# yoxu515/aot-benchmark

Measured on NVIDIA H100. Metric: frames/sec (480p, 10 obj), higher is better.
Workload: dtype f32

## Files before the change

### aot_benchmark_b200/csrc/local_attn.cu

```cuda
#include "common.cuh"

namespace aotb {

constexpr int LW = 15, LR = 7, LTAPS = 225;

__device__ __forceinline__ void cp_async16(float* dst_smem, const float* src, int bytes) {
    asm volatile("cp.async.ca.shared.global [%0], [%1], 16, %2;" ::"r"((uint32_t)__cvta_generic_to_shared(dst_smem)), "l"(src),
                 "r"(bytes) : "memory");
}
__device__ __forceinline__ void cp_async_wait_all() { asm volatile("cp.async.commit_group;\n\tcp.async.wait_group 0;" ::: "memory"); }

struct LocalArgs {
    const float* q; int ldq;
    const float* k; int ldk;
    const float* v; int ldv;
    const float* relk_w;
    const float* relk_b;
    const float* relv;
    float* out; int ldo;
    int h, w, H;
    float T;
};

template <int D, int DV, bool HAS_RELV, bool STAGE_WK>
__global__ void __launch_bounds__(256) local_attn_kernel(const LocalArgs p) {
    pdl_sync();
    constexpr int WARPS = 8;
    constexpr int WKS = D + 4;
    extern __shared__ __align__(16) float smem[];
    float* q_raw = smem;
    float* q_scl = q_raw + WARPS * D;
    float* prob = q_scl + WARPS * D;
    float* wk_s = prob + WARPS * 232;
    float* relv_s = wk_s + (STAGE_WK ? LTAPS * WKS : 0);

    const int g = blockIdx.y;
    const int warp = threadIdx.x >> 5, lane = threadIdx.x & 31;
    const int N = p.h * p.w;
    const int qi = blockIdx.x * WARPS + warp;

    if constexpr (STAGE_WK) {
        const float* src = p.relk_w + (size_t)g * LTAPS * D;
        for (int f = threadIdx.x; f < LTAPS * (D / 4); f += blockDim.x) {
            const int r = f / (D / 4), c = (f % (D / 4)) * 4;
            *reinterpret_cast<float4*>(wk_s + r * WKS + c) = __ldg(reinterpret_cast<const float4*>(src + r * D + c));
        }
    }
    if constexpr (HAS_RELV) {
        const float* src = p.relv + (size_t)g * DV * LTAPS;
        for (int f = threadIdx.x; f < DV * LTAPS; f += blockDim.x) relv_s[f] = __ldg(src + f);
    }
    if (qi < N) {
        for (int c = lane; c < D; c += 32) {
// ... 250 lines not shown
    }
    cp_async_wait_all();
    __syncthreads();

    {
        const int ly = warp / (TX / 3), lx0 = (warp % (TX / 3)) * 3;
        float acc[3] = {0.f, 0.f, 0.f};
#pragma unroll 1
        for (int dy = 0; dy < LW; ++dy) {
            const float* vrow = halo + ((ly + dy) * HWD + lx0) * LD + lane;
            float vv[LW + 2], rr[LW];
#pragma unroll
            for (int j = 0; j < LW + 2; ++j) vv[j] = vrow[j * LD];
#pragma unroll
            for (int dx = 0; dx < LW; ++dx) rr[dx] = rvs[(dy * LW + dx) * D + lane];
#pragma unroll
            for (int i = 0; i < 3; ++i) {
                const float4* pp = reinterpret_cast<const float4*>(prob + (ly * TX + lx0 + i) * PLD + dy * 16);
                const float4 p0 = pp[0], p1 = pp[1], p2 = pp[2], p3 = pp[3];
                const float pa[16] = {p0.x, p0.y, p0.z, p0.w, p1.x, p1.y, p1.z, p1.w,
                                      p2.x, p2.y, p2.z, p2.w, p3.x, p3.y, p3.z, p3.w};
#pragma unroll
                for (int dx = 0; dx < LW; ++dx) acc[i] = fmaf(pa[dx], vv[i + dx] + rr[dx], acc[i]);
            }
        }
        const int y = ty0 + ly;
#pragma unroll
        for (int i = 0; i < 3; ++i) {
            const int x = tx0 + lx0 + i;
            if (y < p.h && x < p.w) p.out[(size_t)(y * p.w + x) * p.ldo + g * D + lane] = acc[i];
        }
    }
}

static int launch_local_tile(const LocalArgs& a, const float* relv_t, cudaStream_t st) {
    constexpr int TY = 8, TX = 6;
    const size_t smem = sizeof(float) * (size_t)((TY + 14) * (TX + 14) * 36 + TY * TX * 32 + TY * TX * LW * 16 + LTAPS * 32);
    static bool configured = false;
    if (!configured) {
        cudaError_t e = cudaFuncSetAttribute(local_attn_tile_kernel<TY, TX>, cudaFuncAttributeMaxDynamicSharedMemorySize,
                                             (int)smem);
        if (e != cudaSuccess) {
            set_error("aotb_local_attention_tile_f32: cudaFuncSetAttribute: %s", cudaGetErrorString(e));
            return AOTB_ERR_CUDA;
        }
        configured = true;
    }
    dim3 grid(cdiv(a.h, TY) * cdiv(a.w, TX), a.H);
    launch(local_attn_tile_kernel<TY, TX>, dim3(grid), dim3(512), smem, st, a, relv_t);
    return check_launch("aotb_local_attention_tile_f32");
}


template <int TY, int TX, int KC, int VC>
__global__ void __launch_bounds__(512, 1) local_gated_tile_kernel(const LocalArgs p) {
    pdl_sync();
    constexpr int C = 32, HH = TY + 2 * LR, HWD = TX + 2 * LR, NPOS = HH * HWD, LD = 36;
    constexpr int NT = 512, NQ = TY * TX, PLD = LW * 16, DQ = KC * C;
    static_assert(TX % 3 == 0 && TY * (TX / 3) == NT / 32, "aggregate pass: one warp per 3 queries");
    static_assert(LW * HWD <= NT && 2 * LTAPS <= NT && NQ % 2 == 0, "pass mappings");
    extern __shared__ __align__(16) float smem[];
    float* halo = smem;
    float* qs = halo + NPOS * LD;
    float* prob = qs + NQ * DQ;

    const int tid = threadIdx.x, warp = tid >> 5, lane = tid & 31;
    const int tiles_x = (p.w + TX - 1) / TX;
    const int ty0 = (blockIdx.x / tiles_x) * TY, tx0 = (blockIdx.x % tiles_x) * TX;
    const int cg = blockIdx.y;

    auto load_halo = [&](const float* src, int ld, int c0) {
        for (int f = tid; f < NPOS * 8; f += NT) {
            const int pos = f >> 3, c4 = (f & 7) * 4;
            const int hy = pos / HWD, hx = pos - hy * HWD;
            const int yy = ty0 - LR + hy, xx = tx0 - LR + hx;
            const bool in = yy >= 0 && yy < p.h && xx >= 0 && xx < p.w;
            cp_async16(halo + pos * LD + c4, in ? src + (size_t)(yy * p.w + xx) * ld + c0 + c4 : src, in ? 16 : 0);
        }
    };
    for (int f = tid; f < NQ * (DQ / 4); f += NT) {
        const int ql = f / (DQ / 4), c4 = (f % (DQ / 4)) * 4;
        const int ly = ql / TX, lx = ql - ly * TX;
        const int y = ty0 + ly, x = tx0 + lx;
        float4 v = make_float4(0.f, 0.f, 0.f, 0.f);
        if (y < p.h && x < p.w) v = __ldg(reinterpret_cast<const float4*>(p.q + (size_t)(y * p.w + x) * p.ldq + c4));
        *reinterpret_cast<float4*>(qs + ql * DQ + c4) = v;
    }
    load_halo(p.k, p.ldk, 0);
    cp_async_wait_all();
    __syncthreads();

    if (tid < 2 * LTAPS) {
        const int half = tid / LTAPS, tap = tid - half * LTAPS;
        const float bias = __ldg(p.relk_b + tap);
        const int slot = (tap / LW) * 16 + tap % LW;
#pragma unroll 1
        for (int kc = 0; kc < KC; ++kc) {
            float wk[C];
            const float4* wp = reinterpret_cast<const float4*>(p.relk_w + (size_t)tap * DQ + kc * C);
#pragma unroll
            for (int c = 0; c < C / 4; ++c) {
                const float4 t = __ldg(wp + c);
                wk[4 * c] = t.x; wk[4 * c + 1] = t.y; wk[4 * c + 2] = t.z; wk[4 * c + 3] = t.w;
            }
#pragma unroll 2
            for (int qi = 0; qi < NQ / 2; ++qi) {
// ... 124 lines not shown

static int launch_local_gated_tile(const LocalArgs& a, cudaStream_t st) {
    constexpr int TY = 8, TX = 6, KC = 4, VC = 8;
    const size_t smem = sizeof(float) * (size_t)((TY + 14) * (TX + 14) * 36 + TY * TX * KC * 32 + TY * TX * LW * 16);
    static bool configured = false;
    if (!configured) {
        cudaError_t e = cudaFuncSetAttribute(local_gated_tile_kernel<TY, TX, KC, VC>, cudaFuncAttributeMaxDynamicSharedMemorySize,
                                             (int)smem);
        if (e != cudaSuccess) {
            set_error("aotb_local_gated_tile_f32: cudaFuncSetAttribute: %s", cudaGetErrorString(e));
            return AOTB_ERR_CUDA;
        }
        configured = true;
    }
    dim3 grid(cdiv(a.h, TY) * cdiv(a.w, TX), 1024 / (VC * 32));
    launch(local_gated_tile_kernel<TY, TX, KC, VC>, dim3(grid), dim3(512), smem, st, a);
    return check_launch("aotb_local_gated_tile_f32");
}

}

using namespace aotb;

extern "C" int aotb_local_attention_f32(const float* q, int ldq, const float* k, int ldk, const float* v, int ldv,
                                        const float* relk_w, const float* relk_b, const float* relv, float* out,
                                        int ldo, int h, int w, int H, int d_att, int d_v, void* stream) {
    AOTB_REQUIRE(q && k && v && relk_w && relk_b && out && h > 0 && w > 0 && H > 0,
                 "aotb_local_attention_f32: bad args");
    AOTB_REQUIRE(ldq % 4 == 0 && ldk % 4 == 0 && ldv % 4 == 0 && ldo % 4 == 0, "aotb_local_attention_f32: ld %% 4");
    LocalArgs a;
    a.q = q; a.ldq = ldq; a.k = k; a.ldk = ldk; a.v = v; a.ldv = ldv;
    a.relk_w = relk_w; a.relk_b = relk_b; a.relv = relv; a.out = out; a.ldo = ldo;
    a.h = h; a.w = w; a.H = H; a.T = sqrtf((float)d_att);
    cudaStream_t st = (cudaStream_t)stream;
    if (d_att == 32 && d_v == 32 && relv) return launch_local<32, 32, true, true>(a, st);
    if (d_att == 128 && d_v == 1024 && !relv) return launch_local<128, 1024, false, false>(a, st);
    set_error("aotb_local_attention_f32: unsupported head shape d_att=%d d_v=%d relv=%d", d_att, d_v, relv != nullptr);
    return AOTB_ERR_UNSUPPORTED;
}

extern "C" int aotb_local_attention_tile_f32(const float* q, int ldq, const float* k, int ldk, const float* v, int ldv,
                                             const float* relk_w, const float* relk_b, const float* relv_t, float* out,
                                             int ldo, int h, int w, int H, void* stream) {
    AOTB_REQUIRE(q && k && v && relk_w && relk_b && relv_t && out && h > 0 && w > 0 && H > 0,
                 "aotb_local_attention_tile_f32: bad args");
    AOTB_REQUIRE(ldq % 4 == 0 && ldk % 4 == 0 && ldv % 4 == 0, "aotb_local_attention_tile_f32: ld %% 4");
    LocalArgs a;
    a.q = q; a.ldq = ldq; a.k = k; a.ldk = ldk; a.v = v; a.ldv = ldv;
    a.relk_w = relk_w; a.relk_b = relk_b; a.relv = nullptr; a.out = out; a.ldo = ldo;
    a.h = h; a.w = w; a.H = H; a.T = sqrtf(32.f);
    return launch_local_tile(a, relv_t, (cudaStream_t)stream);
}

extern "C" int aotb_local_gated_tile_f32(const float* q, int ldq, const float* k, int ldk, const float* v, int ldv,
                                         const float* relk_w, const float* relk_b, float* out, int ldo, int h, int w,
                                         void* stream) {
    AOTB_REQUIRE(q && k && v && relk_w && relk_b && out && h > 0 && w > 0, "aotb_local_gated_tile_f32: bad args");
    AOTB_REQUIRE(ldq % 4 == 0 && ldk % 4 == 0 && ldv % 4 == 0, "aotb_local_gated_tile_f32: ld %% 4");
    LocalArgs a;
    a.q = q; a.ldq = ldq; a.k = k; a.ldk = ldk; a.v = v; a.ldv = ldv;
    a.relk_w = relk_w; a.relk_b = relk_b; a.relv = nullptr; a.out = out; a.ldo = ldo;
    a.h = h; a.w = w; a.H = 1; a.T = sqrtf(128.f);
    return launch_local_gated_tile(a, (cudaStream_t)stream);
}
```

### aot_benchmark_b200/engine.py

```python
from __future__ import annotations

import functools
import math

import numpy as np
import torch
import torch.nn as nn

from . import ops
from .plan import get_plan

A_NONE, A_RELU, A_GELU, A_SILU, A_RELU6 = ops.ACT_NONE, ops.ACT_RELU, ops.ACT_GELU, ops.ACT_SILU, ops.ACT_RELU6
A_HSWISH = ops.ACT_HSWISH

LT_PROBE = None
import os as _os
LT_IMPL = _os.environ.get("AOTB_LT_IMPL", "tc_exact")
LOCAL_IMPL = _os.environ.get("AOTB_LOCAL_IMPL", "tile")
DEAOT_LT = _os.environ.get("AOTB_DEAOT_LT", "tc")
SHARD_XCHG = _os.environ.get("AOTB_SHARD_XCHG", "nccl")
SHARD_SMAX = 16
SUB_ENGINE_STREAMS = _os.environ.get("AOTB_SUB_ENGINE_STREAMS", "1") == "1"
SHARD_GRAPHS = _os.environ.get("AOTB_SHARD_GRAPHS", "1") == "1"


def _symm_alloc(numel, device, group):
    import torch.distributed as dist
    import torch.distributed._symmetric_memory as symm_mem
    t = symm_mem.empty(numel, dtype=torch.float32, device=device)
    hdl = symm_mem.rendezvous(t, group if group is not None else dist.group.WORLD)
    return hdl, (lambda r, sizes, off: hdl.get_buffer(r, sizes, torch.float32, off))


GEMM_GROW_FRAMES = int(_os.environ.get("AOTB_GEMM_GROW_FRAMES", "8"))
_LT_NAMES = {"simt": "attn_f32_kernel<32,32> (fp32 SIMT flash attention)",
             "tc_exact": "attn_tc_kernel<1,1> (wgmma fp16x2 exact: 6+8 MMAs per 64-key tile)",
             "tc_fast": "attn_tc_kernel<1,1> (wgmma fp16 fast: 2+4 MMAs per 64-key tile)"}
_DEAOT_LT_NAMES = {"simt": "attn_f32_kernel<128,256> (fp32 SIMT flash attention, DeAOT 1 x 128 / 1024 head)",
                   "gemm": "conv_tc_kernel (Q K^T) -> row_softmax_kernel -> conv_tc_kernel (P V): wgmma GEMMs over split-fp16 "
                           "copies of the bank (deaot_lt.cu)",
                   "tc": "attn_tc_kernel<4,2> (fused wgmma flash attention, 128 queries x 64 value channels per CTA)"}


def deaot_lt_kernel_name():
    return _DEAOT_LT_NAMES.get(DEAOT_LT, DEAOT_LT)


LT_KERNEL_NAME = _LT_NAMES.get(LT_IMPL, LT_IMPL) + (f", layout '{ops.LT_VARIANT}'" if LT_IMPL.startswith("tc") else "")


USE_GRAPHS = _os.environ.get("AOTB_GRAPHS", "1") == "1"
USE_PDL = _os.environ.get("AOTB_PDL", "1") == "1"
CONV_TILING = _os.environ.get("AOTB_CONV_TILING", "model")
_CONV_TILING_MASK = {"model": 0, "narrow": 1}


def _apply_pdl():
    from ._lib import lib, check
    lib().aotb_set_pdl(1 if USE_PDL else 0)
    check(lib().aotb_set_conv_tiling(_CONV_TILING_MASK[CONV_TILING]), "aotb_set_conv_tiling")
BANK_INIT_FRAMES = int(_os.environ.get("AOTB_BANK_FRAMES", "24"))
OFFLINE_ENC_CHUNK = 16


def _resolve_mem_max(aot_model, long_term_mem_max):
    m = getattr(aot_model.cfg, "TEST_LONG_TERM_MEM_MAX", None) if long_term_mem_max is None else long_term_mem_max
    if m is None:
        return None
    if int(m) != m or m < 2:
        raise ValueError(f"long_term_mem_max must be an integer >= 2 (the first memory frame and at least one recent one), got {m}")
    return int(m)
# ... 951 lines not shown
        for li in range(self._plan().L):
            ops.bank_append(K_src[li], self.bank_K[li], 0, offset_dev=off, stream=st)
            ops.bank_append(V_src[li], self.bank_V[li], 0, offset_dev=off, stream=st)
            if self._tc:
                ops.tc_pack_rows(K_src[li], self.bank_Kp[li], 0, row_off_dev=off, stream=st)
                ops.tc_pack_rows(V_src[li], self.bank_Vp[li], 0, row_off_dev=off, stream=st)
            if self._gemm_lt:
                ops.split_rows(K_src[li], self.bank_Kh[li], self.bank_Kl[li], row_off_dev=off, stream=st)
                ops.split_cols(V_src[li], self.bank_VhT[li], self.bank_VlT[li], col_off_dev=off, stream=st)
            if getattr(self, "_gp_tc", False):
                ops.tc_pack_rows(K_src[li], self.bank_gpK[li], 0, row_off_dev=off, stream=st)
                ops.tc_pack_rows(V_src[li], self.bank_gpV[li], 0, row_off_dev=off, stream=st)
        ops.counter_add(off, N, stream=st)

    def _latest_kv(self):
        return self._new_K, self._new_V

    def _lstt_forward(self, embs, id_emb, st):
        P = self._plan()
        ws = self._ws
        N, C, H = self.enc_hw, P.C, P.H
        h, w = self.enc_size_2d
        d = C // H
        proj = embs.nhwc[-1].view(N, C)
        ops.eltwise(ops.EW_COPY, proj, None, ws.x, stream=st)
        ops.eltwise(ops.EW_COPY, proj, None, ws.cat[:, :C], stream=st)
        x = ws.x
        is_ref = id_emb is not None
        if is_ref:
            stK, stV = self._next_short_slot()
        else:
            stK, stV = self.st_K, self.st_V
        for li in range(P.L):
            Lw = P.layers[li]
            ops.layernorm(x, Lw.norm1[0], Lw.norm1[1], ws.ln, add=self.pos_emb, out2=ws.ln_pos, stream=st)
            ops.linear(ws.ln_pos, Lw.sa_qk_w, Lw.sa_qk_b, ws.qk, stream=st)
            ops.linear(ws.ln, Lw.sa_v_w, Lw.sa_v_b, ws.v, stream=st)
            if self._tc:
                self._tc_attention(ws.qk[:, :C], ws.qk[:, C:], ws.v, None, None, N, ws.core[:, :C], st)
            else:
                ops.attention(ws.qk[:, :C], ws.qk[:, C:], ws.v, ws.core[:, :C], H, d, d, Tk=N, stream=st)
            ops.linear(ws.core[:, :C], Lw.sa_proj_w, Lw.sa_proj_b, x, res=x, stream=st)
            cQ, cV = self.curr_Q[li], self.curr_V[li]
            ops.layernorm(x, Lw.norm2[0], Lw.norm2[1], cV, stream=st)
            ops.linear(cV, Lw.linQ_w, Lw.linQ_b, cQ, stream=st)
            if is_ref:
                ops.eltwise(ops.EW_ADD, cV, id_emb, ws.tmp, stream=st)
                ops.linear(ws.tmp, Lw.linV_w, Lw.linV_b, stV[li], stream=st)
                ops.eltwise(ops.EW_COPY, cQ, None, stK[li], stream=st)
                gK, gV, Tk = stK[li], stV[li], N
            else:
                gK, gV, Tk = self.bank_K[li], self.bank_V[li], self.bank_len
            self._long_term_attention(li, cQ, gK, gV, Tk, ws.core[:, :C], st)
            if d == 32 and LOCAL_IMPL == "tile":
                ops.local_attention_tile(cQ, stK[li], stV[li], Lw.relk_w, Lw.relk_b, Lw.relv_t, ws.core[:, C:], h, w, H,
                                         stream=st)
            else:
                ops.local_attention(cQ, stK[li], stV[li], Lw.relk_w, Lw.relk_b, Lw.relv, ws.core[:, C:], h, w, H, d, d,
                                    stream=st)
            ops.linear(ws.core, Lw.lst_proj_w, Lw.lst_proj_b, x, res=x, stream=st)
            ops.layernorm(x, Lw.norm3[0], Lw.norm3[1], ws.ln, stream=st)
            ops.linear(ws.ln, Lw.lin1_w, Lw.lin1_b, ws.ff, stream=st)
            ops.groupnorm(ws.ff.view(1, N, 4 * C), Lw.gn[0], Lw.gn[1], ws.ff.view(1, N, 4 * C), 32, A_GELU, ws.gn_ws,
                          stream=st)
            ops.dwconv(ws.ff.view(1, h, w, 4 * C), Lw.dw_w, None, ws.ff2.view(1, h, w, 4 * C), K=5, pad=2, stream=st)
            ops.linear(ws.ff2, Lw.lin2_w, Lw.lin2_b, x, res=x, stream=st)
            ops.layernorm(x, Lw.dec_norm[0], Lw.dec_norm[1], ws.cat[:, (li + 1) * C:(li + 2) * C], stream=st)
        if is_ref:
            self._commit_short_slot(stK, stV)
        self._have_lstt = True

    def _long_term_attention(self, li, Q, K, V, Tk, out, st):
        P = self._plan()
        d = P.C // P.H
        probe = LT_PROBE
        use_tc = self._tc and (K is self.bank_K[li])
        if use_tc:
            ops.tc_pack_rows(Q, self._ws.Qp, 0, div=math.sqrt(d), stream=st)
        if probe is not None:
            e0, e1 = torch.cuda.Event(enable_timing=True), torch.cuda.Event(enable_timing=True)
            e0.record()
        if use_tc and self.kv_shard is not None:
            self._sharded_attention(li, out, st)
        elif self.kv_shard is not None and K is self.bank_K[li]:
            raise ops.AotbError("sharded long-term bank needs the tensor-core attention kernel (8 heads x 32); this model's "
                                "head shape runs on the fp32 kernel, which has no partial (m, l, O) outputs")
        elif use_tc and self._usage():
            self._usage_attention(li, self._ws.Qp, self.bank_Kp[li], self.bank_Vp[li], out, st)
        elif use_tc:
            self._tc_attention(None, None, None, self.bank_Kp[li], self.bank_Vp[li], Tk, out, st, Tk_dev=self.tk_dev)
        elif self._tc:
            self._tc_attention(Q, K, V, None, None, Tk, out, st)
        else:
            ops.attention(Q, K, V, out, P.H, d, d, Tk=Tk, Tk_dev=self.tk_dev if K is self.bank_K[li] else None,
                          stream=st)
        if probe is not None:
            e1.record()
            probe.append((e0, e1, 4.0 * Q.shape[0] * Tk * P.C))

    def _tc_attention(self, Q, K, V, Kp, Vp, Tk, out, st, Tk_dev=None):
        P = self._plan()
        ws = self._ws
        d = P.C // P.H
        N = self.enc_hw
        if Q is not None:
            ops.tc_pack_rows(Q, ws.Qp, 0, div=math.sqrt(d), stream=st)
        if Kp is None:
            ops.tc_pack_rows(K, ws.saKp, 0, stream=st)
            ops.tc_pack_rows(V, ws.saVp, 0, stream=st)
# ... 224 lines not shown
        C2, C4 = 2 * C, 4 * C
        proj = embs.nhwc[-1].view(N, C)
        x, z = ws.xz[:, :C], ws.xz[:, C:]
        ops.eltwise(ops.EW_COPY, proj, None, x, stream=st)
        ops.eltwise(ops.EW_FILL, None, None, z, scalar=0.0, stream=st)
        is_ref = id_emb is not None
        if is_ref:
            stK, stV = self._next_short_slot()
        else:
            stK, stV = self.st_K, self.st_V
        for li in range(P.L):
            Lw = P.layers[li]
            cQ, cV = self.curr_Q[li], self.curr_V[li]
            ops.layernorm(x, Lw.norm1[0], Lw.norm1[1], ws.ln, stream=st)
            ops.linear(ws.ln, Lw.qv_w, Lw.qv_b, ws.qv, stream=st)
            ops.eltwise(ops.EW_COPY, ws.qv[:, :d], None, cQ, stream=st)
            ops.eltwise(ops.EW_SILU, ws.qv[:, d:], None, cV, stream=st)
            ops.linear(ws.ln, Lw.u_w, Lw.u_b, ws.catU[:, :C2], act=A_SILU, stream=st)
            if li == 0:
                ops.eltwise(ops.EW_FILL, None, None, ws.catU[:, C2:], scalar=1.0, stream=st)
                cIDV = None
            else:
                cIDV = self.curr_IDV[li]
                ops.layernorm(z, Lw.id_norm1[0], Lw.id_norm1[1], cIDV, stream=st)
                ops.linear(cIDV, Lw.idu_w, Lw.idu_b, ws.catU[:, C2:], act=A_SILU, stream=st)
            if is_ref:
                ops.eltwise(ops.EW_COPY, cQ, None, stK[li], stream=st)
                ops.eltwise(ops.EW_COPY, cV, None, stV[li][:, :C2], stream=st)
                self._fuse_id(li, cIDV, id_emb, stV[li][:, C2:], st)
                gK, gV, Tk = stK[li], stV[li], N
            else:
                gK, gV, Tk = self.bank_K[li], self.bank_V[li], self.bank_len
            probe = LT_PROBE if not is_ref else None
            if probe is not None:
                e0, e1 = torch.cuda.Event(enable_timing=True), torch.cuda.Event(enable_timing=True)
                e0.record()
            if self._gp_tc and not is_ref and self._usage():
                ops.tc_pack_rows(cQ, ws.gpQp, 0, div=math.sqrt(self._kdim), stream=st)
                self._usage_attention(li, ws.gpQp, self.bank_gpK[li], self.bank_gpV[li], ws.core, st)
            elif self._gp_tc and not is_ref:
                self._gp_attention(cQ, None, None, self.bank_gpK[li], self.bank_gpV[li], Tk, self.tk_dev, ws.core, st)
            elif self._gp_tc:
                self._gp_attention(cQ, gK, gV, None, None, N, None, ws.core, st)
            elif self._gemm_lt and not is_ref:
                ops.linear_tc(cQ, self.bank_Kh[li], self.bank_Kl[li], None, ws.S, stream=st)
                ops.row_softmax(ws.S, self._capw, Tk, 1.0 / math.sqrt(d), Tk_dev=self.tk_dev, stream=st)
                ops.linear_tc(ws.S, self.bank_VhT[li], self.bank_VlT[li], None, ws.core, stream=st)
            else:
                ops.attention(cQ, gK, gV, ws.core, 1, d, C4, Tk=Tk, Tk_dev=None if is_ref else self.tk_dev, stream=st)
            if probe is not None:
                e1.record()
                probe.append((e0, e1, 2.0 * N * Tk * (d + C4)))
            self._gated_tail(ws.core, ws.catU, Lw.lt_dw, ws.dw[:, :C4], h, w, st)
            if LOCAL_IMPL == "tile" and d == 128 and C4 == 1024:
                ops.local_gated_tile(cQ, stK[li], stV[li], Lw.relk_w, Lw.relk_b, ws.core, h, w, stream=st)
            else:
                ops.local_attention(cQ, stK[li], stV[li], Lw.relk_w, Lw.relk_b, None, ws.core, h, w, 1, d, C4, stream=st)
            self._gated_tail(ws.core, ws.catU, Lw.st_dw, ws.dw[:, C4:], h, w, st)
            ops.linear(ws.dw, Lw.lst_proj_w, Lw.lst_proj_b, ws.xz, res=ws.xz, stream=st)
            ops.layernorm(x, Lw.norm2[0], Lw.norm2[1], ws.c[:, :C], stream=st)
            ops.layernorm(z, Lw.id_norm2[0], Lw.id_norm2[1], ws.c[:, C:], stream=st)
            ops.linear(ws.c, Lw.sa_qk_w, Lw.sa_qk_b, ws.sa_qk, stream=st)
            ops.linear(ws.c[:, :C], Lw.sa_v1[0], Lw.sa_v1[1], ws.sa_v[:, :C2], act=A_SILU, stream=st)
            ops.linear(ws.c[:, C:], Lw.sa_v2[0], Lw.sa_v2[1], ws.sa_v[:, C2:], act=A_SILU, stream=st)
            ops.linear(ws.c[:, :C], Lw.sa_u1[0], Lw.sa_u1[1], ws.sa_u[:, :C2], act=A_SILU, stream=st)
            ops.linear(ws.c[:, C:], Lw.sa_u2[0], Lw.sa_u2[1], ws.sa_u[:, C2:], act=A_SILU, stream=st)
            if self._gp_tc:
                self._gp_attention(ws.sa_qk, ws.sa_qk, ws.sa_v, None, None, N, None, ws.core, st)
            else:
                ops.attention(ws.sa_qk, ws.sa_qk, ws.sa_v, ws.core, 1, d, C4, Tk=N, stream=st)
            self._gated_tail(ws.core, ws.sa_u, Lw.sa_dw, ws.dw[:, :C4], h, w, st)
            ops.linear(ws.dw[:, :C4], Lw.sa_proj_w, Lw.sa_proj_b, ws.xz, res=ws.xz, stream=st)
        ops.groupnorm(ws.xz.view(1, N, C2), P.final_gn[0], P.final_gn[1], ws.cat.view(1, N, C2), 2, A_NONE, ws.gn_ws,
                      stream=st)
        if is_ref:
            self._commit_short_slot(stK, stV)
        self._have_lstt = True

    def _gp_attention(self, Q, K, V, Kp, Vp, Tk, Tk_dev, out, st):
        ws = self._ws
        N = self.enc_hw
        ops.tc_pack_rows(Q, ws.gpQp, 0, div=math.sqrt(self._kdim), stream=st)
        if Kp is None:
            ops.tc_pack_rows(K, ws.gpSaK, 0, stream=st)
            ops.tc_pack_rows(V, ws.gpSaV, 0, stream=st)
            Kp, Vp = ws.gpSaK, ws.gpSaV
        splits = self._gp_splits(Tk)
        part = None
        if splits > 1:
            part = ws.gp_part.get(splits)
            if part is None:
                fz = lambda *s: torch.empty(s, dtype=torch.float32, device=out.device)
                part = ws.gp_part[splits] = (fz(splits, N, out.shape[1]), fz(splits, 1, N), fz(splits, 1, N))
        ops.gp_attention_tc(ws.gpQp, Kp, Vp, N, Tk, O=out, Tk_dev=Tk_dev, splits=splits, exact=self.precision == "fp32",
                            part=part, stream=st)

    def _gp_splits(self, Tk):
        base = ((self.enc_hw + 127) // 128) * (4 * self._plan().C // 64)
        tiles = (max(Tk, 1) + 63) // 64
        return max(1, min(tiles // 4 if tiles >= 8 else 1, max(1, (2 * 132) // base)))

    def _fuse_id(self, li, cIDV, id_emb, out, st):
        Lw = self._plan().layers[li]
        ws = self._ws
        C = self._plan().C
        if cIDV is None:
            ops.linear(id_emb, Lw.idv_w, Lw.idv_b, out, act=A_SILU, stream=st)
# ... 184 lines not shown
```

### aot_benchmark_b200/ops.py

```python
from __future__ import annotations

import contextlib
import os

import torch

from ._lib import AotbError, check, lib

ACT_NONE, ACT_RELU, ACT_GELU, ACT_SILU, ACT_RELU6, ACT_HSWISH = 0, 1, 2, 3, 4, 5
EW_COPY, EW_ADD, EW_MUL, EW_SILU, EW_SILU_MUL, EW_FILL = 0, 1, 2, 3, 4, 5


def _st(stream):
    return torch.cuda.current_stream().cuda_stream if stream is None else stream


def _chk(*ts):
    for t in ts:
        if t is None:
            continue
        if not t.is_cuda or t.dtype != torch.float32:
            raise AotbError(f"aot_benchmark_b200 kernels need float32 CUDA tensors, got {t.dtype} on {t.device}")
        if t.dim() >= 1 and t.stride(-1) != 1:
            raise AotbError("innermost stride must be 1")
# ... 384 lines not shown
def attn_merge(Opart, Mpart, Lpart, O, H, d_v, stream=None):
    _chk(Opart, Mpart, Lpart, O)
    R, N = Opart.shape[0], Opart.shape[1]
    check(lib().aotb_attn_merge_f32(_p(Opart), _p(Mpart), _p(Lpart), _p(O), R, N, H, d_v, O.stride(0), _st(stream)),
          "aotb_attn_merge_f32")
    return O


def attn_merge_usage_workspace(R, device):
    n = int(lib().aotb_attn_merge_usage_workspace_bytes(int(R)))
    return torch.zeros((n + 7) // 8, dtype=torch.float64, device=device)


def attn_merge_usage(Opart, Mpart, Lpart, O, H, d_v, U, A, live_dev, rows, layers, workspace, stream=None):
    _chk(Opart, Mpart, Lpart, O, U)
    R, N = Opart.shape[0], Opart.shape[1]
    if U.numel() != R or not U.is_contiguous() or (A is not None and (A.dtype != torch.int32 or A.numel() != R or
                                                                      not A.is_cuda)):
        raise AotbError(f"attn_merge_usage: U must be float32 [{R}] and A int32 [{R}] CUDA tensors")
    check(lib().aotb_attn_merge_usage_f32(_p(Opart), _p(Mpart), _p(Lpart), _p(O), R, N, H, d_v, O.stride(0), _p(U), _p(A),
                                          _counter("attn_merge_usage: live_dev", live_dev) if A is not None else None,
                                          int(rows), int(layers), workspace.data_ptr(), _st(stream)),
          "aotb_attn_merge_usage_f32")
    return O


def attn_merge_peers(Oparts, Mparts, Lparts, O, splits, H, d_v, stream=None):
    import ctypes
    _chk(O, *Oparts, *Mparts, *Lparts)
    R, N = len(Oparts), O.shape[0]
    arr = lambda ts: (ctypes.c_void_p * R)(*[t.data_ptr() for t in ts])
    check(lib().aotb_attn_merge_peers_f32(arr(Oparts), arr(Mparts), arr(Lparts), R, int(splits), _p(O), N, H, d_v,
                                          O.stride(0), _st(stream)), "aotb_attn_merge_peers_f32")
    return O


def local_attention(q, k, v, relk_w, relk_b, relv, out, h, w, H, d_att, d_v, stream=None):
    _chk(q, k, v, relk_w, relk_b, relv, out)
    check(lib().aotb_local_attention_f32(_p(q), q.stride(0), _p(k), k.stride(0), _p(v), v.stride(0), _p(relk_w),
                                         _p(relk_b), _p(relv), _p(out), out.stride(0), h, w, H, d_att, d_v,
                                         _st(stream)), "aotb_local_attention_f32")
    return out


def local_gated_tile(q, k, v, relk_w, relk_b, out, h, w, stream=None):
    _chk(q, k, v, relk_w, relk_b, out)
    if q.shape[1] != 128 or k.shape[1] != 128 or v.shape[1] != 1024 or out.shape[1] != 1024 or not relk_w.is_contiguous():
        raise AotbError("local_gated_tile: q / k [hw, 128], v / out [hw, 1024], contiguous relative_emb_k weights [225, 128]")
    check(lib().aotb_local_gated_tile_f32(_p(q), q.stride(0), _p(k), k.stride(0), _p(v), v.stride(0), _p(relk_w), _p(relk_b),
                                          _p(out), out.stride(0), h, w, _st(stream)), "aotb_local_gated_tile_f32")
    return out


def local_attention_tile(q, k, v, relk_w, relk_b, relv_t, out, h, w, H, stream=None):
    _chk(q, k, v, relk_w, relk_b, relv_t, out)
    check(lib().aotb_local_attention_tile_f32(_p(q), q.stride(0), _p(k), k.stride(0), _p(v), v.stride(0), _p(relk_w),
                                              _p(relk_b), _p(relv_t), _p(out), out.stride(0), h, w, H, _st(stream)),
          "aotb_local_attention_tile_f32")
    return out


def _id_embed_check(name, mask, table, table_shape, bias, out, C, ksize, stride, pad, ln_gamma, ln_beta):
    _chk(mask, table, bias, out, ln_gamma, ln_beta)
    if mask.dim() != 2 or not mask.is_contiguous():
        raise AotbError(f"{name}: mask must be a contiguous [Hm, Wm] map, got shape {tuple(mask.shape)}, "
                        f"strides {mask.stride()}")
    Hm, Wm = mask.shape
    ho, wo = (Hm + 2 * pad - ksize) // stride + 1, (Wm + 2 * pad - ksize) // stride + 1
    if tuple(table.shape) != tuple(table_shape) or not table.is_contiguous():
        raise AotbError(f"{name}: weight table must be a contiguous {list(table_shape)}, got {tuple(table.shape)}")
    if bias.numel() != C or any(t is not None and t.numel() != C for t in (ln_gamma, ln_beta)):
        raise AotbError(f"{name}: bias and LayerNorm parameters need {C} entries")
    if out.dim() != 2 or tuple(out.shape) != (ho * wo, C):
        raise AotbError(f"{name}: out must be [{ho * wo}, {C}] for a {Hm}x{Wm} mask, got {tuple(out.shape)}")
    return Hm, Wm


def id_embed(mask, wt, bias, out, C, nid, ksize, stride, pad, ln_gamma=None, ln_beta=None, stream=None):
    Hm, Wm = _id_embed_check("id_embed", mask, wt, (ksize * ksize * nid, C), bias, out, C, ksize, stride, pad, ln_gamma,
                             ln_beta)
    check(lib().aotb_id_embed_f32(_p(mask), Hm, Wm, _p(wt), _p(bias), _p(ln_gamma), _p(ln_beta), _p(out),
                                  out.stride(0), C, nid, ksize, stride, pad, _st(stream)), "aotb_id_embed_f32")
    return out


def id_embed_runs(mask, wp, bias, out, C, nid, ksize, stride, pad, ln_gamma=None, ln_beta=None, stream=None):
    Hm, Wm = _id_embed_check("id_embed_runs", mask, wp, (ksize, ksize + 1, nid, C), bias, out, C, ksize, stride, pad,
                             ln_gamma, ln_beta)
    check(lib().aotb_id_embed_runs_f32(_p(mask), Hm, Wm, _p(wp), _p(bias), _p(ln_gamma), _p(ln_beta), _p(out),
                                       out.stride(0), C, nid, ksize, stride, pad, _st(stream)), "aotb_id_embed_runs_f32")
    return out


def _dense_maps(name, t, shape3):
    if t.dim() < 3 or t.numel() != t.shape[-3] * t.shape[-2] * t.shape[-1] or not t.is_contiguous() \
            or any(want is not None and got != want for got, want in zip(t.shape[-3:], shape3)):
        want = "x".join("*" if v is None else str(v) for v in shape3)
        raise AotbError(f"{name}: need one contiguous [{want}] map, got shape {tuple(t.shape)}, strides {t.stride()}")


def logits_postproc(logits_nhwc, lowres_nchw, out_nchw, obj_num, align_corners, stream=None):
    _chk(logits_nhwc, lowres_nchw, out_nchw)
    _dense_maps("logits_postproc logits", logits_nhwc, (None, None, None))
    h, w, NC = logits_nhwc.shape[-3:]
    _dense_maps("logits_postproc lowres", lowres_nchw, (NC, h, w))
    if out_nchw is not None:
        _dense_maps("logits_postproc out", out_nchw, (NC, None, None))
    Ho, Wo = (out_nchw.shape[-2], out_nchw.shape[-1]) if out_nchw is not None else (0, 0)
    check(lib().aotb_logits_postproc_f32(_p(logits_nhwc), _p(lowres_nchw), _p(out_nchw), h, w, NC, obj_num, Ho, Wo,
                                         1 if align_corners else 0, _st(stream)), "aotb_logits_postproc_f32")
    return out_nchw
# ... 270 lines not shown
```

### include/aotb200.h

```cpp
#ifndef AOTB200_H
#define AOTB200_H
#include <stddef.h>
#ifdef __cplusplus
extern "C" {
#endif

int aotb_version(void);
const char* aotb_arch(void);
const char* aotb_last_error_string(void);
unsigned long long aotb_launch_count(void);
void aotb_set_pdl(int on);
int aotb_set_conv_tiling(int mode);
int aotb_set_conv_grid_cap(int ctas);

int aotb_conv2d_nhwc_f32(const float* in, const float* w, const float* bias, const float* res, float* out,
                         int B, int H, int W, int Cin, int ldin, int Cout, int ldout, int ldres,
                         int KH, int KW, int stride, int pad, int dil, int act, void* stream);

#define AOTB_CONV_CONST_WEIGHTS 256
int aotb_conv2d_nhwc_tc(const float* in, const void* wh, const void* wl, const float* bias, const float* wscale,
                        const float* res, float* out, int B, int H, int W, int Cin, int ldin, int Cout, int ldout, int ldres,
                        int KH, int KW, int stride, int pad, int act, void* workspace, size_t workspace_bytes,
                        void* stream);

// ... 23 lines not shown
int aotb_window_attention_f32(const float* qkv, int ldqkv, const float* qkv_bias, const float* rel_bias, float* out,
                              int ldo, int H, int W, int C, int heads, int window, int shift, void* stream);
int aotb_window_attention_batched_f32(const float* qkv, int ldqkv, const float* qkv_bias, const float* rel_bias, float* out,
                                      int ldo, int B, int H, int W, int C, int heads, int window, int shift, void* stream);

int aotb_patch_merge_f32(const float* x, int ldx, float* out, int ldo, int H, int W, int C, void* stream);
int aotb_patch_merge_batched_f32(const float* x, int ldx, float* out, int ldo, int B, int H, int W, int C, void* stream);

size_t aotb_groupnorm_workspace_bytes(int B, int G);
int aotb_groupnorm_nhwc_f32(const float* x, int ldx, const float* gamma, const float* beta, float* out, int ldo,
                            int B, int P, int C, int G, int act, void* workspace, void* stream);

size_t aotb_splat_workspace_bytes(int C);
int aotb_splat_attention_f32(const float* x, int ldx, int HW, int C, int radix, const float* w1, const float* b1, int inter,
                             const float* w2, const float* b2, float* att, void* workspace, void* stream);
int aotb_splat_combine_f32(const float* x, int ldx, const float* att, float* out, int ldo, int H, int W, int C, int radix,
                           int pool_stride, void* stream);
int aotb_se_gate_f32(const float* x, int ldx, int HW, int C, const float* w1, const float* b1, int inter, const float* w2,
                     const float* b2, float* gate, void* workspace, void* stream);
int aotb_gate_scale_f32(const float* x, int ldx, const float* gate, float* out, int ldo, int HW, int C, int act, void* stream);
size_t aotb_splat_workspace_batched_bytes(int C, int B);
int aotb_splat_attention_batched_f32(const float* x, int ldx, int B, int HW, int C, int radix, const float* w1, const float* b1,
                                     int inter, const float* w2, const float* b2, float* att, void* workspace, void* stream);
int aotb_splat_combine_batched_f32(const float* x, int ldx, const float* att, float* out, int ldo, int B, int H, int W, int C,
                                   int radix, int pool_stride, void* stream);
int aotb_se_gate_batched_f32(const float* x, int ldx, int B, int HW, int C, const float* w1, const float* b1, int inter,
                             const float* w2, const float* b2, float* gate, void* workspace, void* stream);
int aotb_gate_scale_batched_f32(const float* x, int ldx, const float* gate, float* out, int ldo, int B, int HW, int C, int act,
                                void* stream);
int aotb_avgpool_nhwc_f32(const float* in, int ldin, float* out, int ldo, int B, int H, int W, int C, int k, int s, int pad,
                          int ceil_mode, int count_include_pad, void* stream);

int aotb_attention_f32(const float* Q, int ldq, const float* K, int ldk, const float* V, int ldv, float* O,
                       int ldo, int N, int Tk, const int* Tk_dev, int H, int d_qk, int d_v, float* Mout,
                       float* Lout, void* stream);
int aotb_attn_merge_f32(const float* Opart, const float* Mpart, const float* Lpart, float* O, int R, int N,
                        int H, int d_v, int ldo, void* stream);
size_t aotb_attn_merge_usage_workspace_bytes(int R);
int aotb_attn_merge_usage_f32(const float* Opart, const float* Mpart, const float* Lpart, float* O, int R, int N, int H,
                              int d_v, int ldo, float* U, int* A, const int* live, int rows, int layers, void* workspace,
                              void* stream);

int aotb_attn_merge_peers_f32(const void* const* Oparts, const void* const* Mparts, const void* const* Lparts, int ranks,
                              int splits, float* O, int N, int H, int d_v, int ldo, void* stream);

int aotb_local_attention_f32(const float* q, int ldq, const float* k, int ldk, const float* v, int ldv,
                             const float* relk_w, const float* relk_b, const float* relv, float* out, int ldo,
                             int h, int w, int H, int d_att, int d_v, void* stream);

int aotb_local_attention_tile_f32(const float* q, int ldq, const float* k, int ldk, const float* v, int ldv,
                                  const float* relk_w, const float* relk_b, const float* relv_t, float* out, int ldo,
                                  int h, int w, int H, void* stream);

int aotb_local_gated_tile_f32(const float* q, int ldq, const float* k, int ldk, const float* v, int ldv,
                              const float* relk_w, const float* relk_b, float* out, int ldo, int h, int w, void* stream);

int aotb_id_embed_f32(const float* mask, int Hm, int Wm, const float* wt, const float* bias,
                      const float* ln_gamma, const float* ln_beta, float* out, int ldo, int C, int nid,
                      int ksize, int stride, int pad, void* stream);

int aotb_id_embed_runs_f32(const float* mask, int Hm, int Wm, const float* wp, const float* bias,
                           const float* ln_gamma, const float* ln_beta, float* out, int ldo, int C, int nid,
                           int ksize, int stride, int pad, void* stream);

int aotb_logits_postproc_f32(const float* logits_nhwc, float* lowres_nchw, float* out_nchw, int h, int w,
                             int NC, int obj_num, int Ho, int Wo, int align_corners, void* stream);
int aotb_logits_argmax_f32(const float* lowres_nchw, float* label, int h, int w, int NC, int Ho, int Wo,
                           int align_corners, void* stream);
int aotb_soft_logit_aggregation_f32(const float* const* logits, int n_engines, int max_obj, float* out, int HW,
                                    void* stream);
int aotb_separate_labels_f32(const float* mask, int n_engines, int max_obj, float* out, int HW, void* stream);
int aotb_preprocess_bgr_u8(const void* img, int H, int W, const int* ix, const float* cx, const int* iy, const float* cy,
                           float* out, int Ho, int Wo, int flip, void* stream);
int aotb_label_to_u8(const float* label, void* out_u8, int n, void* stream);
int aotb_nearest_resize_f32(const float* in, float* out, int H, int W, int Ho, int Wo, void* stream);
int aotb_tta_merge_f32(const float* const* logits, const int* sizes, const int* flips, int n_augs, int NC, int H, int W,
                       int align_corners, const float* new_label, float* label, float* pred_prob, void* stream);
int aotb_tta_feedback_f32(const float* logits, int h, int w, int NC, int H, int W, int align_corners, int flip,
                          const float* new_label, float* out, int Hi, int Wi, void* stream);

int aotb_tc_pack_rows_f16x2(const float* src, int ld, void* dst, int cap, int rows, int H, int row_off,
                            const int* row_off_dev, float div, void* stream);
size_t aotb_lt_attn_tc_smem_bytes(void);
int aotb_lt_attn_tc_occupancy(int exact, int* ctas_per_sm, int* regs, int* local_bytes);
int aotb_lt_attn_tc_f16x2(const void* Qp, int Nq_cap, const void* Kp, const void* Vp, int kv_cap, int N, int Tk,
                          const int* Tk_dev, int H, float* O, int ldo, float* Opart, float* Mpart, float* Lpart,
                          int splits, int exact, float* dbg, void* stream);
int aotb_lt_attn_tc_slots_f16x2(const void* Qp, int Nq_cap, const void* Kp, const void* Vp, int kv_cap, int N, int Tk,
                                const int* Tk_dev, int H, float* Opart, float* Mpart, float* Lpart, int splits, int split_rows,
                                int exact, void* stream);

int aotb_split_rows_f16x2(const float* src, int lds, void* hi, void* lo, int ldw, int rows, int C, int row_off,
                          const int* row_off_dev, void* stream);
int aotb_split_cols_f16x2(const float* src, int lds, void* hiT, void* loT, int ldt, int rows, int C, int col_off,
                          const int* col_off_dev, void* stream);
int aotb_row_softmax_f32(float* S, int ld, int N, int cols, int Tk, const int* Tk_dev, float scale, void* stream);

int aotb_gp_attn_tc_f16x2(const void* Qp, int Nq_cap, const void* Kp, const void* Vp, int kv_cap, int N, int Tk,
                          const int* Tk_dev, int dv, float* O, int ldo, float* Opart, float* Mpart, float* Lpart,
                          int splits, int exact, void* stream);
int aotb_gp_attn_tc_slots_f16x2(const void* Qp, int Nq_cap, const void* Kp, const void* Vp, int kv_cap, int N, int Tk,
                                const int* Tk_dev, int dv, float* Opart, float* Mpart, float* Lpart, int splits, int split_rows,
                                int exact, void* stream);

int aotb_bank_append_f32(const float* src, int lds, float* bank, int ldb, int rows, int cols, int offset,
                         const int* offset_dev, void* stream);
// ... 14 lines not shown
```

Measured before the change: 400.8.

## Add tensor-core local attention kernel using split-fp16 mma.sync and make it default

Adds a new local (15x15 window) attention kernel for 32-dim heads. It computes QK, the relative-position key bias, softmax and PV with m16n8k16 mma.sync, splitting fp32 operands into hi/lo fp16 with three MMAs each to keep near-fp32 accuracy. It uses an online softmax per window row and stages K and V halos with cp.async, replacing the SIMT tile kernel as the default. The split-precision triple MMA adds conversion overhead and may shift numerics slightly compared with pure fp32.

```diff
diff --git a/aot_benchmark_b200/csrc/local_attn.cu b/aot_benchmark_b200/csrc/local_attn.cu
--- a/aot_benchmark_b200/csrc/local_attn.cu
+++ b/aot_benchmark_b200/csrc/local_attn.cu
@@ -1,4 +1,5 @@
 #include "common.cuh"
+#include "tc_common.cuh"
 
 namespace aotb {
 
@@ -355,6 +356,248 @@
 }
 
 
+constexpr int LTC_TY = 8, LTC_TX = 16, LTC_HH = LTC_TY + 2 * LR, LTC_HW = 32, LTC_LD = 36, LTC_SS = 17;
+constexpr size_t LTC_SMEM = sizeof(float) * (size_t)(2 * LTC_HH * LTC_HW * LTC_LD + LTC_TY * 16 * LTC_SS);
+
+__device__ __forceinline__ void split2(float x, float y, uint32_t& hi, uint32_t& lo) {
+    hi = tc::cvt_h2(x, y);
+    const float2 h = __half22float2(*reinterpret_cast<const __half2*>(&hi));
+    lo = tc::cvt_h2(x - h.x, y - h.y);
+}
+__device__ __forceinline__ void mma16816(float* d, const uint32_t* a, uint32_t b0, uint32_t b1) {
+    asm volatile("mma.sync.aligned.m16n8k16.row.col.f32.f16.f16.f32 {%0, %1, %2, %3}, {%4, %5, %6, %7}, {%8, %9}, "
+                 "{%0, %1, %2, %3};"
+                 : "+f"(d[0]), "+f"(d[1]), "+f"(d[2]), "+f"(d[3])
+                 : "r"(a[0]), "r"(a[1]), "r"(a[2]), "r"(a[3]), "r"(b0), "r"(b1));
+}
+__device__ __forceinline__ void mma_x3(float* d, const uint32_t* ah, const uint32_t* al, const uint32_t* bh, const uint32_t* bl) {
+    mma16816(d, ah, bh[0], bh[1]);
+    mma16816(d, al, bh[0], bh[1]);
+    mma16816(d, ah, bl[0], bl[1]);
+}
+
+__global__ void __launch_bounds__(256, 1) local_attn_mma_kernel(const LocalArgs p, const float* __restrict__ relv_t) {
+    pdl_sync();
+    constexpr int TX = LTC_TX, HW = LTC_HW, LD = LTC_LD, SS = LTC_SS, NPOS = LTC_HH * LTC_HW;
+    extern __shared__ __align__(16) float smem[];
+    float* ks = smem;
+    float* vs = ks + NPOS * LD;
+    const int tid = threadIdx.x, ly = tid >> 5, lane = tid & 31, g4 = lane >> 2, j = lane & 3;
+    float* scr = vs + NPOS * LD + ly * 16 * SS;
+    const int tiles_x = (p.w + TX - 1) / TX;
+    const int ty0 = (blockIdx.x / tiles_x) * LTC_TY, tx0 = (blockIdx.x % tiles_x) * TX;
+    const int g = blockIdx.y;
+
+    for (int f = tid; f < NPOS * 8; f += 256) {
+        const int pos = f >> 3, c4 = (f & 7) * 4;
+        const int yy = ty0 - LR + pos / HW, xx = tx0 - LR + pos % HW;
+        const bool in = yy >= 0 && yy < p.h && xx >= 0 && xx < p.w;
+        const size_t off = (size_t)(yy * p.w + xx);
+        cp_async16(ks + pos * LD + c4, in ? p.k + off * p.ldk + g * 32 + c4 : p.k, in ? 16 : 0);
+        cp_async16(vs + pos * LD + c4, in ? p.v + off * p.ldv + g * 32 + c4 : p.v, in ? 16 : 0);
+    }
+
+    uint32_t qh[2][4], ql[2][4], sh[2][4], sl[2][4];
+    {
+        const int y = ty0 + ly;
+        const float T = p.T;
+#pragma unroll
+        for (int r = 0; r < 2; ++r) {
+            const int x = tx0 + g4 + 8 * r;
+            float4 f[2] = {make_float4(0.f, 0.f, 0.f, 0.f), make_float4(0.f, 0.f, 0.f, 0.f)};
+            if (y < p.h && x < p.w) {
+                const float4* src = reinterpret_cast<const float4*>(p.q + (size_t)(y * p.w + x) * p.ldq + g * 32 + 8 * j);
+                f[0] = __ldg(src);
+                f[1] = __ldg(src + 1);
+            }
+#pragma unroll
+            for (int kk = 0; kk < 2; ++kk) {
+                split2(f[kk].x, f[kk].y, qh[kk][r], ql[kk][r]);
+                split2(f[kk].z, f[kk].w, qh[kk][r + 2], ql[kk][r + 2]);
+                split2(f[kk].x / T, f[kk].y / T, sh[kk][r], sl[kk][r]);
+                split2(f[kk].z / T, f[kk].w / T, sh[kk][r + 2], sl[kk][r + 2]);
+            }
+        }
+    }
+    cp_async_wait_all();
+    __syncthreads();
+
+    const float* wk = p.relk_w + (size_t)g * LTAPS * 32 + 8 * j;
+    const float* bk = p.relk_b + g * LTAPS;
+    const float* rv = relv_t + (size_t)g * LTAPS * 32 + 4 * g4;
+    struct RowOps { float4 wf[2][2]; float b[2][2]; float4 rf[4]; };
+    auto load_row = [&](int dy, RowOps& r) {
+        const float4 z = make_float4(0.f, 0.f, 0.f, 0.f);
+#pragma unroll
+        for (int nt = 0; nt < 2; ++nt) {
+            const int dxb = 8 * nt + g4;
+            const float4* src = reinterpret_cast<const float4*>(wk + (dy * LW + dxb) * 32);
+            r.wf[nt][0] = dxb < LW ? __ldg(src) : z;
+            r.wf[nt][1] = dxb < LW ? __ldg(src + 1) : z;
+#pragma unroll
+            for (int e = 0; e < 2; ++e) {
+                const int dx = 8 * nt + 2 * j + e;
+                r.b[nt][e] = dx < LW ? __ldg(bk + dy * LW + dx) : 0.f;
+            }
+        }
+#pragma unroll
+        for (int t = 0; t < 4; ++t) {
+            const int dx = 2 * j + (t & 1) + 8 * (t >> 1);
+            r.rf[t] = dx < LW ? __ldg(reinterpret_cast<const float4*>(rv + (dy * LW + dx) * 32)) : z;
+        }
+    };
+    RowOps nxt;
+    load_row(0, nxt);
+    float o[4][4] = {};
+    float m[2] = {-INFINITY, -INFINITY}, l[2] = {0.f, 0.f};
+#pragma unroll 1
+    for (int dy = 0; dy < LW; ++dy) {
+        const RowOps cur = nxt;
+        if (dy + 1 < LW) load_row(dy + 1, nxt);
+        const int hr = ly + dy;
+        const int yy = ty0 - LR + hr;
+        const bool yin = yy >= 0 && yy < p.h;
+        float s[2][4];
+#pragma unroll
+        for (int nt = 0; nt < 2; ++nt) {
+#pragma unroll
+            for (int e = 0; e < 2; ++e) {
+                s[nt][e] = cur.b[nt][e];
+                s[nt][e + 2] = cur.b[nt][e];
+            }
+#pragma unroll
+            for (int kk = 0; kk < 2; ++kk) {
+                const float4 f = cur.wf[nt][kk];
+                uint32_t bh[2], bl[2];
+                split2(f.x, f.y, bh[0], bl[0]);
+                split2(f.z, f.w, bh[1], bl[1]);
+                mma_x3(s[nt], qh[kk], ql[kk], bh, bl);
+            }
+        }
+        float sb[4][4] = {};
+#pragma unroll
+        for (int nt = 0; nt < 4; ++nt) {
+            const float4* kp = reinterpret_cast<const float4*>(ks + (hr * HW + 8 * nt + g4) * LD + 8 * j);
+#pragma unroll
+            for (int kk = 0; kk < 2; ++kk) {
+                const float4 f = kp[kk];
+                uint32_t bh[2], bl[2];
+                split2(f.x, f.y, bh[0], bl[0]);
+                split2(f.z, f.w, bh[1], bl[1]);
+                mma_x3(sb[nt], sh[kk], sl[kk], bh, bl);
+            }
+        }
+#pragma unroll
+        for (int nt = 0; nt < 4; ++nt)
+#pragma unroll
+            for (int i = 0; i < 4; ++i) {
+                const int lx = g4 + 8 * (i >> 1), hx = 8 * nt + 2 * j + (i & 1), dx = hx - lx;
+                const int xx = tx0 - LR + hx;
+                if (dx >= 0 && dx < LW) scr[lx * SS + dx] = (yin && xx >= 0 && xx < p.w) ? sb[nt][i] : -1e8f;
+            }
+        __syncwarp();
+        float mx[2] = {m[0], m[1]};
+#pragma unroll
+        for (int nt = 0; nt < 2; ++nt)
+#pragma unroll
+            for (int i = 0; i < 4; ++i) {
+                const int lx = g4 + 8 * (i >> 1), dx = 8 * nt + 2 * j + (i & 1);
+                s[nt][i] = dx < LW ? s[nt][i] + scr[lx * SS + dx] : -INFINITY;
+                mx[i >> 1] = fmaxf(mx[i >> 1], s[nt][i]);
+            }
+        __syncwarp();
+        float sc[2];
+#pragma unroll
+        for (int r = 0; r < 2; ++r) {
+            mx[r] = fmaxf(mx[r], __shfl_xor_sync(0xffffffffu, mx[r], 1));
+            mx[r] = fmaxf(mx[r], __shfl_xor_sync(0xffffffffu, mx[r], 2));
+            sc[r] = expf(m[r] - mx[r]);
+            m[r] = mx[r];
+            l[r] *= sc[r];
+        }
+#pragma unroll
+        for (int nt = 0; nt < 4; ++nt)
+#pragma unroll
+            for (int i = 0; i < 4; ++i) o[nt][i] *= sc[i >> 1];
+#pragma unroll
+        for (int nt = 0; nt < 2; ++nt)
+#pragma unroll
+            for (int i = 0; i < 4; ++i) {
+                s[nt][i] = expf(s[nt][i] - m[i >> 1]);
+                l[i >> 1] += s[nt][i];
+                scr[(g4 + 8 * (i >> 1)) * SS + 8 * nt + 2 * j + (i & 1)] = s[nt][i];
+            }
+        {
+            uint32_t ah[4], al[4];
+            split2(s[0][0], s[0][1], ah[0], al[0]);
+            split2(s[0][2], s[0][3], ah[1], al[1]);
+            split2(s[1][0], s[1][1], ah[2], al[2]);
+            split2(s[1][2], s[1][3], ah[3], al[3]);
+            const float* f0 = &cur.rf[0].x; const float* f1 = &cur.rf[1].x; const float* f2 = &cur.rf[2].x; const float* f3 = &cur.rf[3].x;
+#pragma unroll
+            for (int nt = 0; nt < 4; ++nt) {
+                uint32_t bh[2], bl[2];
+                split2(f0[nt], f1[nt], bh[0], bl[0]);
+                split2(f2[nt], f3[nt], bh[1], bl[1]);
+                mma_x3(o[nt], ah, al, bh, bl);
+            }
+        }
+        __syncwarp();
+#pragma unroll
+        for (int kk = 0; kk < 2; ++kk) {
+            uint32_t ah[4], al[4];
+#pragma unroll
+            for (int t = 0; t < 4; ++t) {
+                const int lx = g4 + 8 * (t & 1), hx = 16 * kk + 2 * j + 8 * (t >> 1);
+                const float p0 = (hx - lx >= 0 && hx - lx < 16) ? scr[lx * SS + hx - lx] : 0.f;
+                const float p1 = (hx + 1 - lx >= 0 && hx + 1 - lx < 16) ? scr[lx * SS + hx + 1 - lx] : 0.f;
+                split2(p0, p1, ah[t], al[t]);
+            }
+            float4 f[4];
+#pragma unroll
+            for (int t = 0; t < 4; ++t)
+                f[t] = *reinterpret_cast<const float4*>(vs + (hr * HW + 16 * kk + 2 * j + (t & 1) + 8 * (t >> 1)) * LD + 4 * g4);
+            const float* f0 = &f[0].x; const float* f1 = &f[1].x; const float* f2 = &f[2].x; const float* f3 = &f[3].x;
+#pragma unroll
+            for (int nt = 0; nt < 4; ++nt) {
+                uint32_t bh[2], bl[2];
+                split2(f0[nt], f1[nt], bh[0], bl[0]);
+                split2(f2[nt], f3[nt], bh[1], bl[1]);
+                mma_x3(o[nt], ah, al, bh, bl);
+            }
+        }
+        __syncwarp();
+    }
+#pragma unroll
+    for (int r = 0; r < 2; ++r) {
+        l[r] += __shfl_xor_sync(0xffffffffu, l[r], 1);
+        l[r] += __shfl_xor_sync(0xffffffffu, l[r], 2);
+        const int y = ty0 + ly, x = tx0 + g4 + 8 * r;
+        if (y < p.h && x < p.w) {
+            const float inv = 1.f / l[r];
+            float4* dst = reinterpret_cast<float4*>(p.out + (size_t)(y * p.w + x) * p.ldo + g * 32 + 8 * j);
+            dst[0] = make_float4(o[0][2 * r] * inv, o[1][2 * r] * inv, o[2][2 * r] * inv, o[3][2 * r] * inv);
+            dst[1] = make_float4(o[0][2 * r + 1] * inv, o[1][2 * r + 1] * inv, o[2][2 * r + 1] * inv, o[3][2 * r + 1] * inv);
+        }
+    }
+}
+
+static int launch_local_tc(const LocalArgs& a, const float* relv_t, cudaStream_t st) {
+    static bool configured = false;
+    if (!configured) {
+        cudaError_t e = cudaFuncSetAttribute(local_attn_mma_kernel, cudaFuncAttributeMaxDynamicSharedMemorySize, (int)LTC_SMEM);
+        if (e != cudaSuccess) {
+            set_error("aotb_local_attention_tc_f32: cudaFuncSetAttribute: %s", cudaGetErrorString(e));
+            return AOTB_ERR_CUDA;
+        }
+        configured = true;
+    }
+    dim3 grid(cdiv(a.h, LTC_TY) * cdiv(a.w, LTC_TX), a.H);
+    launch(local_attn_mma_kernel, grid, dim3(256), LTC_SMEM, st, a, relv_t);
+    return check_launch("aotb_local_attention_tc_f32");
+}
+
+
 template <int TY, int TX, int KC, int VC>
 __global__ void __launch_bounds__(512, 1) local_gated_tile_kernel(const LocalArgs p) {
     pdl_sync();
@@ -585,6 +828,21 @@
     return launch_local_tile(a, relv_t, (cudaStream_t)stream);
 }
 
+extern "C" int aotb_local_attention_tc_f32(const float* q, int ldq, const float* k, int ldk, const float* v, int ldv,
+                                           const float* relk_w, const float* relk_b, const float* relv_t, float* out,
+                                           int ldo, int h, int w, int H, void* stream) {
+    AOTB_REQUIRE(q && k && v && relk_w && relk_b && relv_t && out && h > 0 && w > 0 && H > 0,
+                 "aotb_local_attention_tc_f32: bad args");
+    AOTB_REQUIRE(ldq % 4 == 0 && ldk % 4 == 0 && ldv % 4 == 0 && ldo % 4 == 0, "aotb_local_attention_tc_f32: ld %% 4");
+    AOTB_REQUIRE(((uintptr_t)q | (uintptr_t)k | (uintptr_t)v | (uintptr_t)relk_w | (uintptr_t)relv_t | (uintptr_t)out) % 16 == 0,
+                 "aotb_local_attention_tc_f32: q, k, v, relk_w, relv_t and out must be 16-byte aligned");
+    LocalArgs a;
+    a.q = q; a.ldq = ldq; a.k = k; a.ldk = ldk; a.v = v; a.ldv = ldv;
+    a.relk_w = relk_w; a.relk_b = relk_b; a.relv = nullptr; a.out = out; a.ldo = ldo;
+    a.h = h; a.w = w; a.H = H; a.T = sqrtf(32.f);
+    return launch_local_tc(a, relv_t, (cudaStream_t)stream);
+}
+
 extern "C" int aotb_local_gated_tile_f32(const float* q, int ldq, const float* k, int ldk, const float* v, int ldv,
                                          const float* relk_w, const float* relk_b, float* out, int ldo, int h, int w,
                                          void* stream) {
diff --git a/aot_benchmark_b200/engine.py b/aot_benchmark_b200/engine.py
--- a/aot_benchmark_b200/engine.py
+++ b/aot_benchmark_b200/engine.py
@@ -16,7 +16,7 @@
 LT_PROBE = None
 import os as _os
 LT_IMPL = _os.environ.get("AOTB_LT_IMPL", "tc_exact")
-LOCAL_IMPL = _os.environ.get("AOTB_LOCAL_IMPL", "tile")
+LOCAL_IMPL = _os.environ.get("AOTB_LOCAL_IMPL", "tc")
 DEAOT_LT = _os.environ.get("AOTB_DEAOT_LT", "tc")
 SHARD_XCHG = _os.environ.get("AOTB_SHARD_XCHG", "nccl")
 SHARD_SMAX = 16
@@ -1074,9 +1074,10 @@
             else:
                 gK, gV, Tk = self.bank_K[li], self.bank_V[li], self.bank_len
             self._long_term_attention(li, cQ, gK, gV, Tk, ws.core[:, :C], st)
-            if d == 32 and LOCAL_IMPL == "tile":
-                ops.local_attention_tile(cQ, stK[li], stV[li], Lw.relk_w, Lw.relk_b, Lw.relv_t, ws.core[:, C:], h, w, H,
-                                         stream=st)
+            if d == 32 and LOCAL_IMPL in ops.LOCAL_KERNELS:
+                with ops.local_kernel(LOCAL_IMPL):
+                    ops.local_attention_tile(cQ, stK[li], stV[li], Lw.relk_w, Lw.relk_b, Lw.relv_t, ws.core[:, C:], h, w,
+                                             H, stream=st)
             else:
                 ops.local_attention(cQ, stK[li], stV[li], Lw.relk_w, Lw.relk_b, Lw.relv, ws.core[:, C:], h, w, H, d, d,
                                     stream=st)
@@ -1407,7 +1408,7 @@
                 e1.record()
                 probe.append((e0, e1, 2.0 * N * Tk * (d + C4)))
             self._gated_tail(ws.core, ws.catU, Lw.lt_dw, ws.dw[:, :C4], h, w, st)
-            if LOCAL_IMPL == "tile" and d == 128 and C4 == 1024:
+            if LOCAL_IMPL != "warp" and d == 128 and C4 == 1024:
                 ops.local_gated_tile(cQ, stK[li], stV[li], Lw.relk_w, Lw.relk_b, ws.core, h, w, stream=st)
             else:
                 ops.local_attention(cQ, stK[li], stV[li], Lw.relk_w, Lw.relk_b, None, ws.core, h, w, 1, d, C4, stream=st)
diff --git a/aot_benchmark_b200/ops.py b/aot_benchmark_b200/ops.py
--- a/aot_benchmark_b200/ops.py
+++ b/aot_benchmark_b200/ops.py
@@ -460,11 +460,37 @@
     return out
 
 
+LOCAL_KERNELS = ("tile", "tc")
+_LOCAL_KERNEL = "tile"
+
+
+@contextlib.contextmanager
+def local_kernel(k):
+    global _LOCAL_KERNEL
+    if k not in LOCAL_KERNELS:
+        raise ValueError(f"local kernel must be one of {LOCAL_KERNELS}, got {k!r}")
+    old, _LOCAL_KERNEL = _LOCAL_KERNEL, k
+    try:
+        yield
+    finally:
+        _LOCAL_KERNEL = old
+
+
 def local_attention_tile(q, k, v, relk_w, relk_b, relv_t, out, h, w, H, stream=None):
+    if _LOCAL_KERNEL == "tc":
+        return local_attention_tc(q, k, v, relk_w, relk_b, relv_t, out, h, w, H, stream=stream)
     _chk(q, k, v, relk_w, relk_b, relv_t, out)
     check(lib().aotb_local_attention_tile_f32(_p(q), q.stride(0), _p(k), k.stride(0), _p(v), v.stride(0), _p(relk_w),
                                               _p(relk_b), _p(relv_t), _p(out), out.stride(0), h, w, H, _st(stream)),
           "aotb_local_attention_tile_f32")
+    return out
+
+
+def local_attention_tc(q, k, v, relk_w, relk_b, relv_t, out, h, w, H, stream=None):
+    _chk(q, k, v, relk_w, relk_b, relv_t, out)
+    check(lib().aotb_local_attention_tc_f32(_p(q), q.stride(0), _p(k), k.stride(0), _p(v), v.stride(0), _p(relk_w),
+                                            _p(relk_b), _p(relv_t), _p(out), out.stride(0), h, w, H, _st(stream)),
+          "aotb_local_attention_tc_f32")
     return out
 
 
diff --git a/include/aotb200.h b/include/aotb200.h
--- a/include/aotb200.h
+++ b/include/aotb200.h
@@ -99,6 +99,10 @@
                                   const float* relk_w, const float* relk_b, const float* relv_t, float* out, int ldo,
                                   int h, int w, int H, void* stream);
 
+int aotb_local_attention_tc_f32(const float* q, int ldq, const float* k, int ldk, const float* v, int ldv,
+                                const float* relk_w, const float* relk_b, const float* relv_t, float* out, int ldo,
+                                int h, int w, int H, void* stream);
+
 int aotb_local_gated_tile_f32(const float* q, int ldq, const float* k, int ldk, const float* v, int ldv,
                               const float* relk_w, const float* relk_b, float* out, int ldo, int h, int w, void* stream);
 
```

Measured after the change: 418.7 (median of 6 runs). +4.5%, better.
